# SamsungLabs/Metis

Hardware: NVIDIA H100
Metric: candidate plans evaluated/sec (higher is better)
Workload: dtype f64

## Files before the change

metis_b200/csrc/metis_eval.cuh:

```cuda
#pragma once

#include <stdint.h>
#include <string.h>
#include <math.h>

#include "../../include/metis_b200.h"

#if defined(__CUDACC__)
#define MB_HD __host__ __device__ __forceinline__
#define MB_HD_NOINLINE __host__ __device__ __noinline__
#else
#define MB_HD inline
#define MB_HD_NOINLINE inline
#endif

namespace metis {

constexpr int kH = 7;
constexpr double kMemCoef = 5.0;
constexpr uint8_t kDropped = 0xFF;

struct Tables {
    MetisProblem p;
    const int16_t *key_index;
    const double *lc;
    const double *mem;
    const double *exec_full;
    const double *fb_sync;
    const double *norm_lc;
    const double *type_memory, *bw_first, *bw_min;
    const uint8_t *run_type;
    const int32_t *run_end;
    const int32_t *q10_end;
    const double *dlay;
    const double *inv_exec;
    const double *ratio;
    const double *dpk;
    const double *pp_hidden;
    const double *pp_vocab;
    const double *psub;
    const double *dsub;
    const double *rsum;
};

constexpr int kDpk = 16;

struct DerivedLayout {
    int dlay, inv_exec, ratio, dpk, pp_hidden, pp_vocab, psub, dsub, total;
};

MB_HD DerivedLayout derived_layout(const MetisProblem &p) {
    DerivedLayout d;
    int o = 0;
    d.dlay = o; o += p.norm_len;
    d.inv_exec = o; o += p.num_keys;
    d.ratio = o; o += p.num_layers + 1;
    d.dpk = o; o += kDpk;
    d.pp_hidden = o; o += p.num_bs + 1;
    d.pp_vocab = o; o += (p.num_bs + 1) * p.num_tp;
    d.psub = o; o += (p.norm_len >= p.num_layers) ? kH * p.num_layers + 1 : 0;
    d.dsub = o; o += (p.norm_len >= p.num_layers) ? kH * p.num_layers : 0;
    d.total = o;
    return d;
}

MB_HD double derive_entry(const MetisProblem &p, const DerivedLayout &d, const double *norm_lc,
                          const double *exec_full, const double *bw_first, int i) {
    if (i < d.inv_exec) return norm_lc[i - d.dlay] / 7.0;
    if (i < d.ratio) return 1. / exec_full[i - d.inv_exec];
    if (i < d.dpk) return (double)(i - d.ratio) / (double)p.num_layers;
    const double bw = bw_first[0] * 1048576.0;
    if (i < d.pp_hidden) {
        const int dp = 1 << (i - d.dpk);
        return (double)(2 * (dp - 1)) / ((double)dp * bw);
    }
    if (i < d.pp_vocab) return (double)((int64_t)(i - d.pp_hidden) * p.sequence_length * p.hidden_size) / bw;
    if (i >= d.dsub) return norm_lc[(i - d.dsub) / kH] / 7.0;
    if (i >= d.psub) {
        const int j = i - d.psub, r = j / kH;
        double acc = 0.0;
        for (int t = 0; t < r; ++t) acc += norm_lc[t];
        return r < p.norm_len ? acc + norm_lc[r] * ((double)(j - r * kH) / 7.0) : acc;
    }
    const int e = i - d.pp_vocab;
    const int mbs = e / p.num_tp, tpc = e - mbs * p.num_tp;
    return ((double)((int64_t)mbs * p.sequence_length * p.vocab_size) / (double)(1 << tpc)) / bw;
}

MB_HD void bind_derived(Tables &T, const double *base) {
    const DerivedLayout d = derived_layout(T.p);
    T.dlay = base + d.dlay;
    T.inv_exec = base + d.inv_exec;
    T.ratio = base + d.ratio;
    T.dpk = base + d.dpk;
    T.pp_hidden = base + d.pp_hidden;
    T.pp_vocab = base + d.pp_vocab;
    T.psub = base + d.psub;
    T.dsub = base + d.dsub;
}

struct PlanDesc {
    uint32_t ordinal;
    int ns;
    int S;
    int label;
    int batches;
    const uint8_t *row;
    uint64_t geo;
};

MB_HD uint64_t pack_geo(int64_t row_offset, int S, int label, int ns, int div) {
    return (uint64_t)(row_offset & 0xFFFFFFFFLL) | ((uint64_t)((S - 1) & 0xFF) << 32) | ((uint64_t)((label - 1) & 0xFF) << 40) |
           ((uint64_t)(ns & 0xFF) << 48) | ((uint64_t)(div & 0xFF) << 56);
}

enum BalancerPath {
    kPathVerifyFailed = 0,
    kPathSeqForward = 1,
    kPathIrregular = 2,
    kPathMiddle = 3,
    kPathFirstGe = 4,
    kPathTail = 5,
    kPathVoteEnds = 6,
};

struct Serial {
    static constexpr bool kUniform = false;
    MB_HD void mark(int) const {}
    MB_HD void note(int) const {}
    MB_HD void converge() const {}
    MB_HD void rejoin(bool) {}
};
#if defined(__CUDACC__) && defined(METIS_PROFILE_PHASES)
constexpr int kBulkBatches = 31;
__device__ long long g_bulk_acc[32];
__shared__ long long s_bulk_t[32];
__shared__ int s_bulk_cur[32];
__device__ __forceinline__ void bulk_mark(unsigned group, int id) {
    __syncwarp(group);
    if ((int)(threadIdx.x & 31) == __ffs((int)group) - 1) {
        const int wi = threadIdx.x >> 5;
        const long long now = clock64();
        if (id == 1) atomicAdd((unsigned long long *)&g_bulk_acc[kBulkBatches], 1ULL);
        else atomicAdd((unsigned long long *)&g_bulk_acc[s_bulk_cur[wi] & 31], (unsigned long long)(now - s_bulk_t[wi]));
        s_bulk_cur[wi] = id;
        s_bulk_t[wi] = now;
    }
    __syncwarp(group);
}
#endif
#if defined(__CUDACC__)
struct Lockstep : Serial {
    unsigned mask;
    __device__ Lockstep() : mask(0xFFFFFFFFu) {}
    __device__ void converge() const { __syncwarp(mask); }
    __device__ void rejoin(bool p) { mask = __ballot_sync(0xFFFFFFFFu, p); }
#if defined(METIS_PROFILE_PHASES)
    __device__ void mark(int id) const { bulk_mark(__activemask(), id); }
#endif
};
#endif
struct SerialUniform : Serial {
    static constexpr bool kUniform = true;
};

constexpr uint64_t kOnes = 0x0101010101010101ULL;

constexpr uint16_t kBroke = 0x8000;
constexpr uint16_t kTaken = 0x4000;
constexpr uint16_t kPos = 0x3FFF;

template <int MAXS, int MAXL>
struct Scratch {
    double perf[MAXS];
    double capa[MAXS];
    double mstate[MAXS];
    double extra[MAXS];
    uint16_t fe[MAXS];
    uint16_t first[MAXS], lastl[MAXS], cnt[MAXS];
    uint16_t part[MAXS + 1];
    uint16_t rs[MAXS + 1];
    uint8_t gcode[MAXS];
    uint8_t tpc[MAXS];
    uint8_t lstk[MAXS];
    uint8_t got[MAXS];
    uint64_t ownerw[MAXL / 8 + 1];
    uint64_t subw[MAXL];
    static_assert(MAXL >= MAXS, "after the vote, subw holds one double per stage (CoopEvaluator's adjust and cost)");
};

MB_HD double py_sum_range(const double *x, int a, int b) {
    if (a >= b) return 0.0;
    double f = 0.0 + x[a];
    double c = 0.0;
    for (int i = a + 1; i < b; ++i) {
        const double v = x[i];
        const double t = f + v;
        if (fabs(f) >= fabs(v)) c += (f - t) + v;
        else c += (v - t) + f;
        f = t;
    }
    if (c != 0.0 && isfinite(c)) f += c;
    return f;
}

MB_HD_NOINLINE double py_sum_range_compact(const double *x, int a, int b) {
    if (a >= b) return 0.0;
    double f = 0.0 + x[a];
    double c = 0.0;
#pragma unroll 1
    for (int i = a + 1; i < b; ++i) {
        const double v = x[i];
        const double t = f + v;
        if (fabs(f) >= fabs(v)) c += (f - t) + v;
        else c += (v - t) + f;
        f = t;
    }
    if (c != 0.0 && isfinite(c)) f += c;
    return f;
}

template <class X>
MB_HD double sum_range(const double *x, int a, int b) {
    if constexpr (X::kUniform) return py_sum_range_compact(x, a, b);
    else return py_sum_range(x, a, b);
}

MB_HD void fill_range_sums(const double *row, int L, int a, double *out) {
    const int n = L + 1;
    double f = 0.0 + row[a];
    double c = 0.0;
    out[(size_t)(a + 1) * n + a] = f;
#if defined(__CUDA_ARCH__)
#pragma unroll 1
#endif
    for (int i = a + 1; i < L; ++i) {
        const double v = row[i];
        const double t = f + v;
        if (fabs(f) >= fabs(v)) c += (f - t) + v;
        else c += (v - t) + f;
        f = t;
        out[(size_t)(i + 1) * n + a] = (c != 0.0 && isfinite(c)) ? f + c : f;
    }
}
MB_HD int range_sum_tables(const MetisProblem &p) { return 2 * p.num_keys + 1; }
MB_HD const double *range_sum_row(const MetisProblem &p, int t, const double *mem, const double *lc, const double *norm) {
    if (t < p.num_keys) return mem + (size_t)t * p.lpad;
    if (t < 2 * p.num_keys) return lc + (size_t)(t - p.num_keys) * p.lpad;
    return p.norm_len >= p.num_layers ? norm : nullptr;
}

enum RangeTable { kRangeMem = 0, kRangeLc = 1, kRangeNorm = 2 };
template <class X>
MB_HD double range_sum(const Tables &T, int family, int key, const double *row, int a, int b) {
    if (a >= b) return 0.0;
    if (T.rsum && b <= T.p.num_layers) {
        const int n = T.p.num_layers + 1;
        const int t = family == kRangeMem ? key : family == kRangeLc ? T.p.num_keys + key : 2 * T.p.num_keys;
#if defined(__CUDA_ARCH__)
        return __ldg(&T.rsum[((size_t)t * n + b) * n + a]);
#else
        return T.rsum[((size_t)t * n + b) * n + a];
#endif
    }
    return sum_range<X>(row, a, b);
}

struct PySum {
    double f, c;
    int n;
    MB_HD PySum() : f(0.0), c(0.0), n(0) {}
    MB_HD void add(double v) {
        if (n == 0) { f = 0.0 + v; }
        else {
            const double t = f + v;
            if (fabs(f) >= fabs(v)) c += (f - t) + v;
            else c += (v - t) + f;
            f = t;
        }
        ++n;
    }
    MB_HD double result() const {
        double r = f;
        if (c != 0.0 && isfinite(c)) r += c;
        return r;
    }
};

MB_HD double pow2_neg(int k) {
    const uint64_t bits = (uint64_t)(1023 - k) << 52;
    double d;
    memcpy(&d, &bits, sizeof(d));
    return d;
}

MB_HD int type_of_rank(const Tables &T, int ns, int rank) {
    const int nt = T.p.num_types;
    const int32_t *end = T.run_end + ns * nt;
    const uint8_t *typ = T.run_type + ns * nt;
#pragma unroll 1
    for (int k = 0; k < nt; ++k)
        if (rank < end[k]) return typ[k];
    return typ[nt - 1];
}

MB_HD int type_of_q10(const Tables &T, int ns, int idx) {
    const int nt = T.p.num_types;
    const int32_t *end = T.q10_end + ns * nt;
    const uint8_t *typ = T.run_type + ns * nt;
#pragma unroll 1
    for (int k = 0; k < nt; ++k)
        if (idx < end[k]) return typ[k];
    return typ[nt - 1];
}

MB_HD int key_of(const Tables &T, int type, int tpc, int bs) {
    if (tpc >= T.p.num_tp || bs < 1 || bs > T.p.num_bs) return -1;
    return T.key_index[(type * T.p.num_tp + tpc) * T.p.num_bs + (bs - 1)];
}

template <int MAXS, int MAXL>
MB_HD int fwd_start(const Scratch<MAXS, MAXL> &w, int s) {
    if (s == 0) return 0;
    const uint16_t e = w.fe[s - 1];
    return (e & kPos) + ((e & kBroke) ? 1 : 0);
}

template <int MAXS, int MAXL>
MB_HD bool fwd_nonempty(const Scratch<MAXS, MAXL> &w, int s) {
    return (int)(w.fe[s] & kPos) > fwd_start(w, s);
}

MB_HD int popc64(uint64_t v) {
#if defined(__CUDA_ARCH__)
    return __popcll(v);
#else
    return __builtin_popcountll(v);
#endif
}
MB_HD int ctz64(uint64_t v) {
#if defined(__CUDA_ARCH__)
    return __ffsll((long long)v) - 1;
#else
    return __builtin_ctzll(v);
#endif
}
MB_HD int popc32(uint32_t v) {
#if defined(__CUDA_ARCH__)
    return __popc(v);
#else
    return __builtin_popcount(v);
#endif
}
MB_HD int ctz32(uint32_t v) {
#if defined(__CUDA_ARCH__)
    return __ffs((int)v) - 1;
#else
    return __builtin_ctz(v);
#endif
}
MB_HD int clz32(uint32_t v) {
#if defined(__CUDA_ARCH__)
    return __clz((int)v);
#else
    return __builtin_clz(v);
#endif
}
MB_HD int clz64(uint64_t v) {
#if defined(__CUDA_ARCH__)
    return __clzll((long long)v);
#else
    return __builtin_clzll(v);
#endif
}

MB_HD uint64_t swar_eq(uint64_t x, int c) {
    const uint64_t y = x ^ ((uint64_t)c * kOnes);
    const uint64_t lo7 = 0x7F7F7F7F7F7F7F7FULL;
    return ~((((y & lo7) + lo7) | y) | lo7);
}

MB_HD int swar_count(uint64_t x, int c) { return popc64(swar_eq(x, c) & 0x0080808080808080ULL); }

MB_HD int layer_owner(uint64_t v, bool plurality) {
    if (plurality) {
        int best = 0, own = (int)kDropped;
#pragma unroll 1
        for (int q = 0; q < kH; ++q) {
            const int cq = (int)((v >> (8 * q)) & 0xFF);
            const int n = swar_count(v, cq);
            if (n > best || (n == best && cq < own)) { best = n; own = cq; }
        }
        return own;
    }
    const int c3 = (int)((v >> 24) & 0xFF);
    if (swar_count(v, c3) * 2 > kH) return c3;
    const int c0 = (int)(v & 0xFF), c1 = (int)((v >> 8) & 0xFF), c2 = (int)((v >> 16) & 0xFF);
    if (swar_count(v, c0) * 2 > kH) return c0;
    if (c1 != c0 && swar_count(v, c1) * 2 > kH) return c1;
    if (c2 != c1 && c2 != c0 && swar_count(v, c2) * 2 > kH) return c2;
    return (int)kDropped;
}

template <int MAXS, int MAXL, class X>
MB_HD int balance_run(const Tables &T, int S, Scratch<MAXS, MAXL> &w, const X &x) {
    const int L = T.p.num_layers;
    if (T.p.norm_len < L) return METIS_FATAL_INDEX;
    const double *dlay = T.dlay;
    const double *lc = T.norm_lc;
    const int N = kH * L;
    const int lim = (N - 1 - kH) > 0 ? (N - 1 - kH) : 0;
    const int last = S - 1;
    int broken = METIS_FATAL_NONE;

#pragma unroll (X::kUniform ? 1 : 0)
    for (int s = 0; s < S; ++s) { w.got[s] = 0; w.cnt[s] = 0; }

    x.mark(10);
    int k = 0, sTop = -1;
    bool topSkip = false;
    if (S > 1) {
        int s = 0, j = 0;
        double c = w.perf[0];
#pragma unroll (X::kUniform ? 1 : 0)
        for (int r = 0; r + 1 < L; ++r) {
            const double d = dlay[r];
            const int nsub = (r == L - 2) ? kH - 1 : kH;
#pragma unroll
            for (int q = 0; q < kH; ++q) {
                if (q < nsub) {
                    if (s < last) {
                        if (c > d) {
                            c -= d;
                        } else {
                            w.capa[s] = c;
                            w.fe[s] = (uint16_t)(j | kBroke);
                            ++s;
                            c = w.perf[s];
                        }
                    }
                    ++j;
                }
            }
        }
        if (s < last) {
            x.note(kPathTail);
            w.capa[s] = c;
            w.fe[s] = (uint16_t)lim;
#pragma unroll (X::kUniform ? 1 : 0)
            for (int t = s + 1; t < last; ++t) { w.capa[t] = w.perf[t]; w.fe[t] = (uint16_t)lim; }
            k = lim;
            sTop = s;
        } else {
            k = (w.fe[last - 1] & kPos) + 1;
            sTop = last - 1;
            topSkip = true;
        }
    }

    x.mark(11);
    x.converge();
    int m;
    {
        double c = w.perf[last];
        const double dl = dlay[L - 1];
#pragma unroll (X::kUniform ? 1 : 0)
        for (int i = 0; i < kH; ++i) c -= dl;
        m = N - kH;
        int sp = S - 2;
#pragma unroll (X::kUniform ? 1 : 0)
        while (m > 0) {
            const int j = m - 1;
            bool un = (j >= k);
            if (!un) {
#pragma unroll (X::kUniform ? 1 : 0)
                while (sp >= 0 && (!(w.fe[sp] & kBroke) || (int)(w.fe[sp] & kPos) > j)) --sp;
                un = (sp >= 0 && (int)(w.fe[sp] & kPos) == j);
            }
            if (!un) break;
            const double d = dlay[j / kH];
            if (!(c > d)) break;
            c -= d;
            m = j;
            if (j < k) w.fe[sp] |= kTaken;
        }
        w.capa[last] = c;
    }

    x.mark(12);
    x.converge();
    {
        int start = 0;
#pragma unroll (X::kUniform ? 1 : 0)
        for (int s = 0; s < last; ++s) {
            const uint16_t e = w.fe[s];
            const int pos = e & kPos;
            const int next_start = pos + ((e & kBroke) ? 1 : 0);
            if ((e & (kBroke | kTaken)) != kBroke) { start = next_start; continue; }
            const int j = pos;
            int lo = 0;
            if (pos > start) {
                lo = s;
            } else {
                x.note(kPathIrregular);
#pragma unroll (X::kUniform ? 1 : 0)
                for (int u = s;; --u) {
                    if (u < s) {
                        const int t = w.lstk[u];
                        const bool above = (t == last) || (fwd_nonempty(w, t) && fwd_start(w, t) > j);
                        if (!above) { lo = t; break; }
                    }
                    if (fwd_nonempty(w, u)) { lo = u; break; }
                    if (u == 0) break;
                }
            }
            int hi = s + 1;
            if (hi < last && !((int)(w.fe[hi] & kPos) > next_start && !w.got[hi])) {
                ++hi;
#pragma unroll (X::kUniform ? 1 : 0)
                while (hi < last && (!fwd_nonempty(w, hi) || w.got[hi])) ++hi;
            }
            if (lo > hi) { broken = METIS_FATAL_SCRATCH; hi = lo; }
            int pick = lo;
            double best = w.capa[lo];
#pragma unroll (X::kUniform ? 1 : 0)
            for (int t = lo + 1; t <= hi; ++t)
                if (w.capa[t] > best) { best = w.capa[t]; pick = t; }
            w.capa[pick] -= dlay[j / kH];
            w.lstk[s] = (uint8_t)pick;
            w.got[pick] = 1;
            start = next_start;
        }
    }
    x.converge();
    const int nblk = m - k;
    if (nblk > 0) x.note(kPathMiddle);
    uint8_t *mid = reinterpret_cast<uint8_t *>(w.subw);
    {
        int below = -1;
#pragma unroll (X::kUniform ? 1 : 0)
        for (int t = 0; t < nblk; ++t) {
            const int j = k + t;
            int lo = 0;
            if (below >= 0) lo = below;
            else if (sTop >= 0) {
#pragma unroll (X::kUniform ? 1 : 0)
                for (int u = sTop;; --u) {
                    if (u < sTop || topSkip) {
                        const uint16_t eu = w.fe[u];
                        if ((eu & (kBroke | kTaken)) == kBroke) {
                            const int t2 = w.lstk[u];
                            if (t2 != last) { lo = t2; break; }
                        }
                    }
                    if (fwd_nonempty(w, u)) { lo = u; break; }
                    if (u == 0) break;
                }
            }
            int pick = lo;
            double best = w.capa[lo];
#pragma unroll (X::kUniform ? 1 : 0)
            for (int t2 = lo + 1; t2 <= last; ++t2)
                if (w.capa[t2] > best) { best = w.capa[t2]; pick = t2; }
            w.capa[pick] -= dlay[j / kH];
            if (pick != last) below = pick;
            mid[t] = (uint8_t)pick;
        }
    }

    x.mark(13);
    x.converge();
    if (k > 0) x.note(kPathVoteEnds);
    int t = 0, nxt = 0;
    uint16_t e = 0;
    if (k > 0) { e = w.fe[0]; nxt = (int)(e & kPos) + ((e & kBroke) ? 1 : 0); }
    const bool plurality = (T.p.corrected & METIS_FIX_Q5) != 0;
    int run_own = (int)kDropped, run_first = 0, run_len = 0;
#pragma unroll (X::kUniform ? 1 : 0)
    for (int r = 0; r < L; ++r) {
        int own = last;
        if (kH * r < m) {
            uint64_t v = 0xFF00000000000000ULL;
#pragma unroll
            for (int q = 0; q < kH; ++q) {
                const int j = kH * r + q;
                int st = last;
                if (j < k) {
#pragma unroll 1
                    while (nxt <= j) { ++t; e = w.fe[t]; nxt = (int)(e & kPos) + ((e & kBroke) ? 1 : 0); }
                    st = t;
                    if (nxt - 1 == j && (e & kBroke)) st = (e & kTaken) ? last : (int)w.lstk[t];
                } else if (j < m) {
                    st = mid[j - k];
                }
                v |= (uint64_t)(uint32_t)st << (8 * q);
            }
            own = layer_owner(v, plurality);
        }
        reinterpret_cast<uint8_t *>(w.ownerw)[r] = (uint8_t)own;
        {
            if (own == run_own) ++run_len;
            else {
                if (run_own != (int)kDropped) {
                    if (w.cnt[run_own] == 0) w.first[run_own] = (uint16_t)run_first;
                    w.lastl[run_own] = (uint16_t)(r - 1);
                    w.cnt[run_own] = (uint16_t)(w.cnt[run_own] + run_len);
                }
                run_own = own; run_first = r; run_len = 1;
            }
        }
    }
    if (run_own != (int)kDropped) {
        if (w.cnt[run_own] == 0) w.first[run_own] = (uint16_t)run_first;
        w.lastl[run_own] = (uint16_t)(L - 1);
        w.cnt[run_own] = (uint16_t)(w.cnt[run_own] + run_len);
    }
    x.mark(14);
    x.converge();
    uint8_t *owner = reinterpret_cast<uint8_t *>(w.ownerw);
    int top = 0x7FFFFFFF;
    double maxc = -INFINITY;
#pragma unroll (X::kUniform ? 1 : 0)
    for (int s = 0; s < S; ++s) {
        const double c = w.cnt[s] ? w.perf[s] - range_sum<X>(T, kRangeNorm, 0, lc, w.first[s], (int)w.lastl[s] + 1) : w.perf[s];
        w.capa[s] = c;
        if (c > maxc) { maxc = c; top = s; }
    }

    x.mark(15);
    x.converge();
#pragma unroll (X::kUniform ? 1 : 0)
    for (int n = 1; n <= 3; ++n) {
        if (top == 0x7FFFFFFF) top = 0;
        int nb = -1;
        double val = INFINITY;
        if (top - 1 >= 0 && w.capa[top - 1] < val) { nb = top - 1; val = w.capa[top - 1]; }
        if (top + 1 < S && w.capa[top + 1] < val) { nb = top + 1; }
        if (nb < 0 || w.cnt[nb] <= 1) break;
        const int layer = (top > nb) ? w.lastl[nb] : w.first[nb];
        const double dl = lc[layer];
        const double ntop = w.capa[top] - dl;
        const double nnb = w.capa[nb] + dl;
        double newmax = -INFINITY;
        int newtop = 0x7FFFFFFF;
#pragma unroll (X::kUniform ? 1 : 0)
        for (int t = 0; t < S; ++t) {
            const double v = (t == top) ? ntop : (t == nb) ? nnb : w.capa[t];
            if (v > newmax) { newmax = v; newtop = t; }
        }
        if (newmax > maxc) break;
        owner[layer] = (uint8_t)top;
        w.capa[top] = ntop;
        w.capa[nb] = nnb;
        if (top > nb) { int r = layer - 1; while (owner[r] != nb) --r; w.lastl[nb] = (uint16_t)r; }
        else          { int r = layer + 1; while (owner[r] != nb) ++r; w.first[nb] = (uint16_t)r; }
        if (w.cnt[top] == 0) { w.first[top] = (uint16_t)layer; w.lastl[top] = (uint16_t)layer; }
        else {
            if (layer < (int)w.first[top]) w.first[top] = (uint16_t)layer;
            if (layer > (int)w.lastl[top]) w.lastl[top] = (uint16_t)layer;
        }
        ++w.cnt[top];
        --w.cnt[nb];
        maxc = newmax;
        top = newtop;
    }

    x.mark(16);
    x.converge();
    w.part[0] = 0;
#pragma unroll (X::kUniform ? 1 : 0)
    for (int s = 0; s < S; ++s) w.part[s + 1] = (uint16_t)(w.part[s] + w.cnt[s]);
    return broken;
}

struct HSplit {
    int nruns;
    int type[METIS_MAX_TYPES];
    int n[METIS_MAX_TYPES];
    int base[METIS_MAX_TYPES];
    int plus[METIS_MAX_TYPES];
};

MB_HD_NOINLINE int partition_data(const Tables &T, int ns, int rank_lo, int count, int dp, int tpc, int bs,
                                  HSplit &out, uint32_t &aux, bool q10 = false) {
    const int gsz = count / dp;
    double perf[METIS_MAX_TYPES];
    PySum total;
    out.nruns = 0;
#pragma unroll 1
    for (int i = 0; i < dp; ++i) {
        const int t = q10 ? type_of_q10(T, ns, rank_lo + i * gsz) : type_of_rank(T, ns, rank_lo + i * gsz);
        if (out.nruns == 0 || out.type[out.nruns - 1] != t) {
            const int key = key_of(T, t, tpc, 1);
            if (key < 0) { aux = ((uint32_t)tpc << 16) | 1u; return METIS_FATAL_KEY_EXEC; }
            const double e = T.exec_full[key];
            if (e == 0.0) return METIS_FATAL_ZERODIV;
            out.type[out.nruns] = t;
            out.n[out.nruns] = 0;
            perf[out.nruns] = 1. / e;
            ++out.nruns;
        }
        ++out.n[out.nruns - 1];
        total.add(perf[out.nruns - 1]);
    }
    const double tot = total.result();
    double frac[METIS_MAX_TYPES];
    int assigned = 0;
#pragma unroll 1
    for (int r = 0; r < out.nruns; ++r) {
        const double v = (double)bs * (perf[r] / tot);
        const int b = (int)v;
        out.base[r] = b;
        out.plus[r] = 0;
        frac[r] = v - (double)b;
        assigned += b * out.n[r];
    }
    int rem = bs - assigned;
    bool used[METIS_MAX_TYPES];
#pragma unroll 1
    for (int r = 0; r < out.nruns; ++r) used[r] = false;
#pragma unroll 1
    for (int it = 0; it < out.nruns && rem > 0; ++it) {
        int pick = -1;
#pragma unroll 1
        for (int r = 0; r < out.nruns; ++r)
            if (!used[r] && (pick < 0 || frac[r] > frac[pick])) pick = r;
        used[pick] = true;
        const int g = rem < out.n[pick] ? rem : out.n[pick];
        out.plus[pick] = g;
        rem -= g;
    }
    if (rem > 0) return METIS_FATAL_SCRATCH;
    return METIS_FATAL_NONE;
}


struct TraceTap {
    double *demand;
    double *state;
    double cost[5];
};

MB_HD int halvings_of(const MetisProblem &p, int S, const uint8_t *gcode, const uint8_t *tpc, int bs_total) {
    int ltp = 0, lbs = 0;
    while ((2 << ltp) <= p.max_tp) ++ltp;
    while ((2 << lbs) <= p.max_bs) ++lbs;
    int u = 0;
#if defined(__CUDA_ARCH__)
#pragma unroll 1
#endif
    for (int s = 0; s < S; ++s) {
        const int g = gcode[s], t = tpc[s];
        int lm = 0;
        while ((2 << lm) <= (bs_total >> (g - t))) ++lm;
        int room = g - t;
        if (ltp - t < room) room = ltp - t;
        if (lbs - lm < room) room = lbs - lm;
        if (room > 0) u += room;
    }
    return u;
}

MB_HD double encode_error(int rc, uint32_t aux) { return rc ? (double)rc + (double)aux * 256.0 : 0.0; }
MB_HD int decode_error(double word, uint32_t &aux) {
    const uint64_t code = (uint64_t)word;
    aux = (uint32_t)(code >> 8);
    return (int)(code & 0xFF);
}

template <int MAXS, int MAXL, class X = Serial, bool ONE = false>
struct PlanEvaluator {
    const Tables &T;
    Scratch<MAXS, MAXL> &w;
    X x;
    PlanDesc pd;
    int bs_total;
    int nbad;
    uint32_t aux;
    TraceTap *tap;

    MB_HD PlanEvaluator(const Tables &t, Scratch<MAXS, MAXL> &s, const X &lanes = X())
        : T(t), w(s), x(lanes), bs_total(0), nbad(0), aux(0), tap(nullptr) {}

    MB_HD int group(int s) const { return 1 << w.gcode[s]; }
    MB_HD int dp_of(int s) const { return (1 << w.gcode[s]) >> w.tpc[s]; }

    MB_HD bool stage_bad(int g, int t) const {
        const int mbs = bs_total >> (g - t);
        return mbs == 0 || mbs > T.p.max_bs || (1 << t) > T.p.max_tp;
    }

    MB_HD int begin(const PlanDesc &plan) {
        pd = plan;
        if (pd.S > MAXS || T.p.num_layers > MAXL) return -1;
        bs_total = T.p.gbs / pd.batches;
        int lb = 0;
#pragma unroll (X::kUniform ? 1 : 0)
        while ((2 << lb) <= bs_total) ++lb;
        nbad = 0;
        int a = 0;
        for (int s = 0; s < pd.S; ++s) {
            const int g = pd.row[s];
            const int t = g > lb ? g - lb : 0;
            if (stage_bad(g, t)) { nbad = 1; return 0; }
            w.gcode[s] = (uint8_t)g;
            w.rs[s] = (uint16_t)a;
            a += 1 << g;
            w.tpc[s] = (uint8_t)t;
        }
        w.rs[pd.S] = (uint16_t)a;
        return nbad == 0 ? 1 : 0;
    }

    MB_HD bool next_strategy(bool have_state) {
        int pick = -1;
        if (have_state) {
            double best = 0.0;
#pragma unroll (X::kUniform ? 1 : 0)
            for (int s = 0; s < pd.S; ++s)
                if (w.gcode[s] != w.tpc[s] && (pick < 0 || w.mstate[s] < best)) { pick = s; best = w.mstate[s]; }
        } else {
            int best = -1;
#pragma unroll (X::kUniform ? 1 : 0)
            for (int s = 0; s < pd.S; ++s) {
                const int ldp = (int)w.gcode[s] - (int)w.tpc[s];
                if (ldp != 0 && ldp > best) { pick = s; best = ldp; }
            }
        }
        if (pick < 0) return false;
        const int g = w.gcode[pick], t = w.tpc[pick];
        nbad += (stage_bad(g, t + 1) ? 1 : 0) - (stage_bad(g, t) ? 1 : 0);
        w.tpc[pick] = (uint8_t)(t + 1);
        return true;
    }

    MB_HD bool valid() const { return nbad == 0; }

    MB_HD int halvings() const { return halvings_of(T.p, pd.S, w.gcode, w.tpc, bs_total); }

    MB_HD double memory_capacity(int a, int b) const {
        const int nt = T.p.num_types;
        if (ONE || nt == 1) return T.type_memory[0] * (double)(b - a);
        const int32_t *end = T.run_end + pd.ns * nt;
        const uint8_t *typ = T.run_type + pd.ns * nt;
        PySum acc;
        int lo = 0;
#pragma unroll (X::kUniform ? 1 : 0)
        for (int k = 0; k < nt; ++k) {
            const int hi = end[k];
            const int x = (a > lo ? a : lo), y = (b < hi ? b : hi);
            if (y > x) acc.add(T.type_memory[typ[k]] * (double)(y - x));
            lo = hi;
        }
        return acc.result();
    }

    MB_HD int replica_perf_cost(int type, int tpc, int h, double &out) {
        double acc = 0.;
#pragma unroll (X::kUniform ? 1 : 0)
        for (int bit = 30; bit >= 0; --bit) {
            const int piece = 1 << bit;
            if (!(h & piece)) continue;
            const int key = key_of(T, type, tpc, piece);
            if (key < 0) { aux = ((uint32_t)tpc << 16) | (uint32_t)piece; return METIS_FATAL_KEY_EXEC; }
            acc += T.exec_full[key];
        }
        out = acc;
        return 0;
    }

    MB_HD_NOINLINE int hetero_performance(int a, int b, int dp, int tpc, double &p) {
        HSplit hs;
        int rc = partition_data(T, pd.ns, a, b - a, dp, tpc, bs_total, hs, aux);
        if (rc) return rc;
        double mx = -INFINITY;
#pragma unroll (X::kUniform ? 1 : 0)
        for (int r = 0; r < hs.nruns; ++r) {
            double c;
            if (hs.plus[r] > 0) {
                rc = replica_perf_cost(hs.type[r], tpc, hs.base[r] + 1, c);
                if (rc) return rc;
                if (c > mx) mx = c;
            }
            if (hs.plus[r] < hs.n[r]) {
                rc = replica_perf_cost(hs.type[r], tpc, hs.base[r], c);
                if (rc) return rc;
                if (c > mx) mx = c;
            }
        }
        p = (mx != 0.0) ? 1. / mx : 0.0;
        return 0;
    }

    MB_HD int rank_start(int s) const { return w.rs[s]; }


    MB_HD int stage_performance(int s, double &p) {
        const int g = w.gcode[s], tpc = w.tpc[s];
        const int a = rank_start(s), b = a + (1 << g);
        int ta = 0, tb = 0;
        if (!(ONE || T.p.num_types == 1)) { ta = type_of_rank(T, pd.ns, a); tb = type_of_rank(T, pd.ns, b - 1); }
        p = 0.0;
        if (ta != tb) return hetero_performance(a, b, 1 << (g - tpc), tpc, p);
        const int bs = bs_total >> (g - tpc);
        const int key = key_of(T, ta, tpc, bs);
        if (key < 0) { aux = ((uint32_t)tpc << 16) | (uint32_t)bs; return METIS_FATAL_KEY_EXEC; }
        if (T.exec_full[key] == 0.0) return METIS_FATAL_ZERODIV;
        p = T.inv_exec[key];
        return 0;
    }

    MB_HD int stage_memory(int s, double &demand, double &state) {
        const bool one_type = ONE || T.p.num_types == 1;
        const bool own_type = (T.p.corrected & METIS_FIX_Q6) != 0;
        const int g = w.gcode[s], tpc = w.tpc[s];
        const int a = rank_start(s), b = a + (1 << g);
        int rc = 0;
        demand = 0.001;
        if (!ONE && own_type) {
            rc = memory_demand_own_type(s, demand);
        } else if (T.p.q10_devices < T.p.total_devices && !own_type && b > T.p.q10_devices) {
            aux = 0;
            rc = METIS_FATAL_INDEX;
        } else if (one_type || type_of_q10(T, pd.ns, a) == type_of_q10(T, pd.ns, b - 1)) {
            const int bs = bs_total >> (g - tpc);
            const int key = key_of(T, T.run_type[pd.ns * T.p.num_types], tpc, bs);
            if (key < 0) { aux = ((uint32_t)tpc << 16) | (uint32_t)bs; rc = METIS_FATAL_KEY_MEMORY; }
            else demand += range_sum<X>(T, kRangeMem, key, T.mem + (size_t)key * T.p.lpad, w.part[s], w.part[s + 1]) * kMemCoef;
        } else {
            rc = hetero_memory_demand(s, T.run_type[pd.ns * T.p.num_types], demand);
        }
        state = memory_capacity(a, b) - demand;
        return rc;
    }

    MB_HD void stage_adjust(int s, double &avail, double &adj, double &extra) const {
        const double c = w.perf[s], md = w.extra[s];
        const double mc = memory_capacity(rank_start(s), rank_start(s) + group(s));
        if (mc > md) {
            adj = c;
            avail = (c * mc / md) - c;
            extra = 0.0;
        } else {
            avail = 0.0;
            adj = c * (mc / md) * 0.9;
            extra = c - adj;
        }
    }

    MB_HD bool stage_time(int s, double &len) {
        const bool one_type = ONE || T.p.num_types == 1;
        const int g = w.gcode[s], tpc = w.tpc[s];
        const int a = one_type ? 0 : rank_start(s), b = a + (1 << g);
        const int la = w.part[s], lb = w.part[s + 1];
        const int ldp = g - tpc;
        const int ta = one_type ? 0 : type_of_rank(T, pd.ns, a);
        const int tb = one_type ? 0 : type_of_rank(T, pd.ns, b - 1);
        len = 0.0;
        if (ta != tb) return hetero_exec_cost(a, b, 1 << ldp, tpc, la, lb, len) != 0;
        const int key = key_of(T, ta, tpc, bs_total >> ldp);
        if (key < 0) return true;
        len = range_sum<X>(T, kRangeLc, key, T.lc + (size_t)key * T.p.lpad, la, lb);
        return false;
    }

    MB_HD void stage_terms(int s, int nstage, double &pp, double &dpc, double &upd) const {
        const int per = T.p.devices_per_node;
        const int Lm = T.p.num_layers;
        const bool ubw = T.p.uniform_bw != 0;
        const int g = w.gcode[s], tpc = w.tpc[s];
        const int la = w.part[s], lb = w.part[s + 1];
        const int ldp = g - tpc;
        const int mbs = bs_total >> ldp;
        const double inv_tp = pow2_neg(tpc);
        pp = 0.0;
        if (s < nstage - 1) {
            if (ubw) {
                pp = (lb == Lm - 1) ? T.pp_vocab[mbs * T.p.num_tp + tpc] : T.pp_hidden[mbs];
            } else {
                double act;
                if (lb == Lm - 1)
                    act = (double)((int64_t)mbs * T.p.sequence_length * T.p.vocab_size) * inv_tp;
                else
                    act = (double)((int64_t)mbs * T.p.sequence_length * T.p.hidden_size);
                pp = act / (bw_of_node_range(rank_start(s) / per, (rank_start(s + 2) - 1) / per) * 1048576.0);
            }
        }
        int ntr = lb - la;
        double params = 0.0;
        if (la == 0) { params += T.p.input_params * inv_tp; --ntr; }
        if (lb == Lm) { params += T.p.output_params * inv_tp; --ntr; }
        params += T.p.transformer_params * inv_tp * (double)ntr;
        if (ubw) dpc = T.dpk[ldp] * params;
        else {
            const int dp = 1 << ldp;
            dpc = (double)(2 * (dp - 1)) / ((double)dp * (dp_bandwidth(rank_start(s), dp, 1 << tpc) * 1048576.0)) * params;
        }
        upd = T.p.optimizer_time * inv_tp * T.ratio[lb - la];
    }


    MB_HD int compute_performance() {
        PySum total;
        int rc = 0;
#pragma unroll (X::kUniform ? 1 : 0)
        for (int s = 0; s < pd.S; ++s) {
            double p;
            rc = stage_performance(s, p);
            if (rc) break;
            w.perf[s] = p;
            total.add(p);
        }
        x.converge();
        if (rc) return rc;
        const double tot = total.result();
        if (tot == 0.0) return METIS_FATAL_ZERODIV;
#pragma unroll (X::kUniform ? 1 : 0)
        for (int s = 0; s < pd.S; ++s) w.perf[s] = w.perf[s] / tot;
        return 0;
    }

    MB_HD_NOINLINE int hetero_memory_demand(int s, int type0, double &demand) {
        const int la = w.part[s], lb = w.part[s + 1], tpc = w.tpc[s];
        HSplit hs;
        const int rc = partition_data(T, pd.ns, 0, T.p.q10_devices, dp_of(s), tpc, bs_total, hs, aux, true);
        if (rc) return rc;
#pragma unroll (X::kUniform ? 1 : 0)
        for (int r = 0; r < hs.nruns; ++r)
#pragma unroll (X::kUniform ? 1 : 0)
            for (int i = 0; i < hs.n[r]; ++i) {
                const int h = hs.base[r] + (i < hs.plus[r] ? 1 : 0);
#pragma unroll (X::kUniform ? 1 : 0)
                for (int bit = 30; bit >= 0; --bit) {
                    const int piece = 1 << bit;
                    if (!(h & piece)) continue;
                    const int key = key_of(T, type0, tpc, piece);
                    if (key < 0) { aux = ((uint32_t)tpc << 16) | (uint32_t)piece; return METIS_FATAL_KEY_MEMORY; }
                    demand += range_sum<X>(T, kRangeMem, key, T.mem + (size_t)key * T.p.lpad, la, lb) * kMemCoef;
                }
            }
        return 0;
    }

    MB_HD_NOINLINE int memory_demand_own_type(int s, double &demand) {
        const int la = w.part[s], lb = w.part[s + 1], tpc = w.tpc[s], g = w.gcode[s];
        const int a = rank_start(s), b = a + (1 << g);
        const int ta = type_of_rank(T, pd.ns, a), tb = type_of_rank(T, pd.ns, b - 1);
        if (ta == tb) {
            const int bs = bs_total >> (g - tpc);
            const int key = key_of(T, ta, tpc, bs);
            if (key < 0) { aux = ((uint32_t)tpc << 16) | (uint32_t)bs; return METIS_FATAL_KEY_MEMORY; }
            demand += range_sum<SerialUniform>(T, kRangeMem, key, T.mem + (size_t)key * T.p.lpad, la, lb) * kMemCoef;
            return 0;
        }
        HSplit hs;
        const int rc = partition_data(T, pd.ns, a, b - a, 1 << (g - tpc), tpc, bs_total, hs, aux);
        if (rc) return rc;
        double worst = 0.0;
#pragma unroll 1
        for (int r = 0; r < hs.nruns; ++r)
#pragma unroll 1
            for (int v = 0; v < 2; ++v) {
                const int cntv = v ? hs.plus[r] : hs.n[r] - hs.plus[r];
                const int h = hs.base[r] + v;
                if (cntv <= 0 || h == 0) continue;
                double need = 0.0;
#pragma unroll 1
                for (int bit = 30; bit >= 0; --bit) {
                    const int piece = 1 << bit;
                    if (!(h & piece)) continue;
                    const int key = key_of(T, hs.type[r], tpc, piece);
                    if (key < 0) { aux = ((uint32_t)tpc << 16) | (uint32_t)piece; return METIS_FATAL_KEY_MEMORY; }
                    need += range_sum<SerialUniform>(T, kRangeMem, key, T.mem + (size_t)key * T.p.lpad, la, lb) * kMemCoef;
                }
                if (need > worst) worst = need;
            }
        demand += worst;
        return 0;
    }

    MB_HD_NOINLINE int adjust_performance() {
        const int S = pd.S;
        double need = 0.;
        PySum avail_sum;
#pragma unroll (X::kUniform ? 1 : 0)
        for (int s = 0; s < S; ++s) {
            double av, adj, extra;
            stage_adjust(s, av, adj, extra);
            w.capa[s] = av;
            w.mstate[s] = adj;
            w.extra[s] = 0.;
            need += extra;
            avail_sum.add(av);
        }
        if (avail_sum.result() < need) return 1;
        int guard = 0;
#pragma unroll (X::kUniform ? 1 : 0)
        while (need > 0.01) {
            PySum tot;
#pragma unroll (X::kUniform ? 1 : 0)
            for (int s = 0; s < S; ++s) tot.add(w.capa[s] > 0.001 ? w.perf[s] : 0.0);
            const double tmp_total = tot.result();
#pragma unroll (X::kUniform ? 1 : 0)
            for (int s = 0; s < S; ++s) {
                const double av = w.capa[s];
                const double ratio = av > 0.001 ? w.perf[s] / tmp_total : 0.0;
                const double want = need * ratio;
                const double give = want > av ? av : want;
                w.extra[s] += give;
                w.capa[s] -= give;
                need -= give;
            }
            if (++guard > 4096) return -METIS_FATAL_HANG;
        }
#pragma unroll (X::kUniform ? 1 : 0)
        for (int s = 0; s < S; ++s) w.perf[s] = w.extra[s] + w.mstate[s];
        return 0;
    }

    MB_HD int memory_phase(int attempt) {
        const int S = pd.S;
        bool oom = false;
        int rc = 0;
#pragma unroll (X::kUniform ? 1 : 0)
        for (int s = 0; s < S; ++s) {
            double md, state;
            rc = stage_memory(s, md, state);
            if (rc) break;
            w.extra[s] = md;
            w.mstate[s] = state;
            if (state < 0) oom = true;
            if (tap) { tap->demand[s] = md; tap->state[s] = state; }
        }
        x.converge();
        if (rc) return -rc;
        if (!oom) return 1;
        if (attempt >= 3) return 0;
        x.mark(21);
        const int adj = adjust_performance();
        if (adj < 0) return adj;
        return adj == 1 ? 0 : 2;
    }

    template <class Sink>
    MB_HD_NOINLINE int partition_layer(Sink &sink) {
#pragma unroll (X::kUniform ? 1 : 0)
        for (int attempt = 1; attempt <= 3; ++attempt) {
            sink.balancer_run();
            const int rc = balance_run<MAXS, MAXL>(T, pd.S, w, x);
            if (rc) return -rc;
            const int r = memory_phase(attempt);
            if (r == 1) return attempt;
            if (r <= 0) return r;
        }
        return 0;
    }

    MB_HD double bw_of_node_range(int n0, int n1) const {
        const int per = T.p.devices_per_node;
        if (n0 == n1) return T.bw_first[type_of_q10(T, pd.ns, n0 * per)];
        double slow = INFINITY;
        const int nt = T.p.num_types;
        const int32_t *end = T.q10_end + pd.ns * nt;
        const uint8_t *typ = T.run_type + pd.ns * nt;
        int lo = 0;
#pragma unroll (X::kUniform ? 1 : 0)
        for (int k = 0; k < nt; ++k) {
            const int hi = end[k];
            if (hi > lo && n0 * per < hi && (n1 + 1) * per > lo) {
                const double v = T.bw_min[typ[k]];
                if (v < slow) slow = v;
            }
            lo = hi;
        }
        return slow;
    }

    MB_HD double dp_bandwidth(int a, int dp, int tp) const {
        const int per = T.p.devices_per_node;
        double slow = INFINITY;
#pragma unroll (X::kUniform ? 1 : 0)
        for (int d = 0; d < dp; ++d) {
            const int n0 = (a + d) / per;
            int nlast = n0;
            bool multi = false;
            double gmin = INFINITY;
            int tprev = -1;
#pragma unroll (X::kUniform ? 1 : 0)
            for (int i = 0; i < tp; ++i) {
                const int node = (a + d + i * dp) / per;
                if (node != nlast) { multi = true; nlast = node; }
                const int t = type_of_q10(T, pd.ns, node * per);
                if (t != tprev) { const double v = T.bw_min[t]; if (v < gmin) gmin = v; tprev = t; }
            }
            const double bw = multi ? gmin : T.bw_first[type_of_q10(T, pd.ns, n0 * per)];
            if (bw < slow) slow = bw;
        }
        return slow;
    }

    MB_HD_NOINLINE int hetero_exec_cost(int a, int b, int dp, int tpc, int la, int lb, double &len) {
        HSplit hs;
        uint32_t dummy;
        if (partition_data(T, pd.ns, a, b - a, dp, tpc, bs_total, hs, dummy)) return 1;
        len = -INFINITY;
#pragma unroll (X::kUniform ? 1 : 0)
        for (int r = 0; r < hs.nruns; ++r)
#pragma unroll (X::kUniform ? 1 : 0)
            for (int v = 0; v < 2; ++v) {
                const int cntv = v ? hs.plus[r] : hs.n[r] - hs.plus[r];
                const int h = hs.base[r] + v;
                if (cntv <= 0 || h == 0) continue;
                double acc = 0.;
#pragma unroll (X::kUniform ? 1 : 0)
                for (int bit = 30; bit >= 0; --bit) {
                    const int piece = 1 << bit;
                    if (!(h & piece)) continue;
                    if (piece > T.p.max_bs) return 1;
                    const int key = key_of(T, hs.type[r], tpc, piece);
                    if (key < 0) return 1;
                    acc += range_sum<X>(T, kRangeLc, key, T.lc + (size_t)key * T.p.lpad, la, lb);
                }
                if (acc > len) len = acc;
            }
        return 0;
    }

    MB_HD int fb_sync_cost(int a, int b, int tpc, int mbs, double &out) const {
        const int nt = T.p.num_types;
        const int32_t *end = T.run_end + pd.ns * nt;
        const uint8_t *typ = T.run_type + pd.ns * nt;
        double mx = -INFINITY;
        int lo = 0;
#pragma unroll (X::kUniform ? 1 : 0)
        for (int k = 0; k < nt; ++k) {
            const int hi = end[k];
            if ((a > lo ? a : lo) < (b < hi ? b : hi)) {
                const int key = key_of(T, typ[k], tpc, mbs);
                if (key < 0) return 1;
                const double v = T.fb_sync[key];
                if (v == 0.0) return 1;
                if (v > mx) mx = v;
            }
            lo = hi;
        }
        out = mx;
        return 0;
    }

    MB_HD int get_cost(double &cost_out) {
        const bool one_type = ONE || T.p.num_types == 1;
        const int nstage = pd.label < pd.S ? pd.label : pd.S;
        if (T.p.q10_devices < T.p.total_devices && rank_start(nstage) > T.p.q10_devices) return 1;
        bool bad = false;
        PySum lens_sum;
        double max_len = -INFINITY;
#pragma unroll (X::kUniform ? 1 : 0)
        for (int s = 0; s < nstage; ++s) {
            double len;
            if (stage_time(s, len)) bad = true;
            lens_sum.add(len);
            if (len > max_len) max_len = len;
        }
        if (bad) return 1;
        double max_upd = -INFINITY, max_dp = -INFINITY;
        double pp_cost = 0., fb_sync = 0.;
#pragma unroll (X::kUniform ? 1 : 0)
        for (int s = 0; s < nstage; ++s) {
            double pp, dpc, upd;
            stage_terms(s, nstage, pp, dpc, upd);
            if (s < nstage - 1) pp_cost += pp;
            if (dpc > max_dp) max_dp = dpc;
            if (upd > max_upd) max_upd = upd;
        }
        {
            const int s = nstage - 1;
            const int a = one_type ? 0 : rank_start(s), b = a + group(s);
            double v;
            if (fb_sync_cost(a, b, w.tpc[s], bs_total >> (w.gcode[s] - w.tpc[s]), v)) return 1;
            fb_sync = v * (double)pd.batches;
        }
        const double exec = ((double)(pd.batches - 1) * max_len) + lens_sum.result();
        const double bg = T.p.batch_generator * (double)pd.batches;
        cost_out = exec + fb_sync + max_upd + max_dp + pp_cost + bg;
        if (tap) { tap->cost[0] = exec; tap->cost[1] = fb_sync; tap->cost[2] = max_upd; tap->cost[3] = max_dp; tap->cost[4] = pp_cost; }
        return 0;
    }

    template <class Sink>
    MB_HD_NOINLINE void run(const PlanDesc &plan, Sink &sink, int only_step = -1) {
        const int ok = begin(plan);
        if (ok < 0) { sink.fatal(plan.ordinal, METIS_FATAL_SCRATCH, 0); return; }
        if (ok == 0) return;
        bool started = false, have_state = false;
        int nrep = 0, step = 0;
#pragma unroll (X::kUniform ? 1 : 0)
        for (;;) {
            if (nrep == 1) return;
            int attempt = 0;
#pragma unroll (X::kUniform ? 1 : 0)
            for (;;) {
                if (!started) started = true;
                else if (!next_strategy(have_state)) return;
                if (!valid()) continue;
                sink.partition_call();
                int rc = compute_performance();
                if (rc) { sink.fatal(pd.ordinal, rc, aux); return; }
                attempt = partition_layer(sink);
                if (attempt < 0) { sink.fatal(pd.ordinal, -attempt, aux); return; }
                have_state = attempt > 0;
                if (attempt > 0) break;
            }
            nrep = attempt;
            double cost;
            if (get_cost(cost) == 0) sink.emit(pd, step, nrep, cost, w.tpc, w.part);
            else sink.keyerror();
            if (only_step >= 0 && step == only_step) return;
            ++step;
        }
    }
};

template <int MAXS, int MAXL, bool ONE, class X = Serial, class Sink>
MB_HD bool first_task(const Tables &T, Scratch<MAXS, MAXL> &w, Sink &sink, bool has, const PlanDesc &plan, int &chain_hint,
                      int &resume) {
    PlanEvaluator<MAXS, MAXL, X, ONE> ev(T, w);
    bool cont = false;
    sink.phase(1);
    if (has) {
        const int ok = ev.begin(plan);
        if (ok < 0) sink.fatal(plan.ordinal, METIS_FATAL_SCRATCH, 0);
        has = ok == 1;
    }
    ev.x.rejoin(has);
    if (has) {
        sink.partition_call();
        const int rc = ev.compute_performance();
        if (rc) { sink.fatal(plan.ordinal, rc, ev.aux); has = false; }
    }
    sink.phase(2);
    ev.x.rejoin(has);
    if (has) {
        sink.balancer_run();
        const int rc = balance_run<MAXS, MAXL>(T, plan.S, w, ev.x);
        if (rc) { sink.fatal(plan.ordinal, rc, ev.aux); has = false; }
    }
    sink.phase(3);
    ev.x.rejoin(has);
    bool costing = false;
    if (has) {
        const int r = ev.memory_phase(1);
        if (r < 0) sink.fatal(plan.ordinal, -r, ev.aux);
        else if (r != 1) {
            cont = true;
            chain_hint = ev.halvings();
            resume = r == 2 ? 2 : 3;
        } else costing = true;
    }
    sink.phase(4);
    ev.x.rejoin(costing);
    if (costing) {
        double cost;
        if (ev.get_cost(cost) == 0) sink.emit(plan, 0, 1, cost, w.tpc, w.part);
        else sink.keyerror();
    }
    sink.phase(0);
    ev.x.rejoin(true);
    return cont;
}

MB_HD int homo_cost(const Tables &T, int type, int dp, int pp, int tp, int mbs, int gbs, double &cost_out,
                    int &oom, TraceTap *tap = nullptr) {
    const int L = T.p.num_layers;
    const int per = T.p.devices_per_node;
    int tpc = 0;
#pragma unroll 1
    while ((1 << tpc) < tp) ++tpc;
    const int key = ((1 << tpc) == tp) ? key_of(T, type, tpc, mbs) : -1;
    if (key < 0) return 1;
    const int num_mbs = gbs / mbs / dp;
    (void)type;
    const double intra = T.p.node0_bandwidth;
    const double inter = T.p.node0_bandwidth;
    const int base = (L - 2) / pp, rem = (L - 2) % pp;
    PySum lens_sum;
    double max_len = -INFINITY, max_params = -INFINITY, max_mem = -INFINITY;
    double pp_cost = 0., fb_sync = 0.;
    int a = 0;
#pragma unroll 1
    for (int s = 0; s < pp; ++s) {
        int count = base + ((s >= 1 && s <= rem) ? 1 : 0) + (s == 0 ? 1 : 0) + (s == pp - 1 ? 1 : 0);
        const int b = a + count;
        const double len = py_sum_range(T.lc + (size_t)key * T.p.lpad, a, b);
        lens_sum.add(len);
        if (len > max_len) max_len = len;
        PySum ps;
#pragma unroll 1
        for (int r = a; r < b && r < L; ++r) {
            const double v = (r == 0) ? T.p.input_params / (double)tp
                           : (r == L - 1) ? T.p.output_params / (double)tp
                           : T.p.transformer_params / (double)tp;
            ps.add(v);
        }
        const double sp = ps.result();
        if (sp > max_params) max_params = sp;
        const double sm = py_sum_range(T.mem + (size_t)key * T.p.lpad, a, b);
        if (sm > max_mem) max_mem = sm;
        if (tap) tap->demand[s] = sm;
        if (s == pp - 1) {
            const double v = T.fb_sync[key];
            if (v == 0.0) return 1;
            fb_sync = v * (double)num_mbs;
        } else {
            double act;
            if (b == L - 1) act = (double)((int64_t)mbs * T.p.sequence_length * T.p.vocab_size) / (double)tp;
            else act = (double)((int64_t)mbs * T.p.sequence_length * T.p.hidden_size);
            double bw = intra;
#pragma unroll 1
            for (int d = 0; d < dp; ++d)
#pragma unroll 1
                for (int t = 0; t < tp; ++t) {
                    const int r0 = s * dp * tp + d * tp + t, r1 = r0 + dp * tp;
                    if (r0 / per != r1 / per) bw = inter;
                }
            pp_cost += act / (bw * 1048576.0);
        }
        a = b;
    }
    oom = (T.p.node0_memory < max_mem) ? 1 : 0;
    const double exec = ((double)(num_mbs - 1) * max_len) + lens_sum.result();
    const double upd = T.p.optimizer_time / (double)pp / (double)tp;
    double bw = intra;
#pragma unroll 1
    for (int p = 0; p < pp; ++p)
        if ((p * dp * tp) / per != ((p + 1) * dp * tp - 1) / per) bw = inter;
    const double dpc = (double)(2 * (dp - 1)) / ((double)dp * (bw * 1048576.0)) * max_params;
    const double bg = T.p.batch_generator * (double)num_mbs;
    cost_out = exec + fb_sync + upd + dpc + pp_cost + bg;
    if (tap) { tap->cost[0] = exec; tap->cost[1] = fb_sync; tap->cost[2] = upd; tap->cost[3] = dpc; tap->cost[4] = pp_cost; }
    return 0;
}

}
```

Baseline: 210.5 million.

## Prefetch stage capacities and vote slots ahead in balance loops

Adds a small lookahead buffer (Ahead) so that the next perf values and fe/lstk vote slots are loaded into registers before they are needed. The stage-assignment loop becomes branch-free selects, with a noinline fallback used when more than two stages advance within one layer. The run-length accounting uses a register bitmask of seen stages instead of reading w.cnt. The aim is to take dependent local-memory loads off the critical path and cut divergence, at the cost of extra registers and some redundant loads.

Result: no change. 211.5 million (median of 6 runs) (+0.5%).

```diff
diff --git a/metis_b200/csrc/metis_eval.cuh b/metis_b200/csrc/metis_eval.cuh
--- a/metis_b200/csrc/metis_eval.cuh
+++ b/metis_b200/csrc/metis_eval.cuh
@@ -402,6 +402,26 @@
     return (int)kDropped;
 }
 
+template <class V>
+struct Ahead {
+    V n1, n2, f3, f4;
+    template <class At> MB_HD void init(const At &at) { n1 = at(1); n2 = at(2); f3 = at(3); f4 = at(4); }
+    template <class At> MB_HD void advance(int moved, int i, const At &at) {
+        if (moved == 1) { n1 = n2; n2 = f3; }
+        else if (moved == 2) { n1 = f3; n2 = f4; }
+        else if (moved > 2) { n1 = at(i + 1); n2 = at(i + 2); }
+        if (moved > 0) { f3 = at(i + 3); f4 = at(i + 4); }
+    }
+    MB_HD V next(int moved) const { return moved == 0 ? n1 : n2; }
+};
+
+template <class At>
+MB_HD_NOINLINE auto ahead_miss(const At &at, int i) -> decltype(at(i)) { return at(i); }
+
+struct VoteSlot {
+    uint32_t fe, lk;
+};
+
 template <int MAXS, int MAXL, class X>
 MB_HD int balance_run(const Tables &T, int S, Scratch<MAXS, MAXL> &w, const X &x) {
     const int L = T.p.num_layers;
@@ -420,28 +440,35 @@
     int k = 0, sTop = -1;
     bool topSkip = false;
     if (S > 1) {
-        int s = 0, j = 0;
+        int s = 0, sh = 0, j = 0;
         double c = w.perf[0];
+        const auto perf_at = [&](int i) { return w.perf[i < last ? i : last]; };
+        Ahead<double> pa;
+        pa.init(perf_at);
+        double d = dlay[0];
 #pragma unroll (X::kUniform ? 1 : 0)
         for (int r = 0; r + 1 < L; ++r) {
-            const double d = dlay[r];
+            const double dn = dlay[r + 1];
             const int nsub = (r == L - 2) ? kH - 1 : kH;
+            pa.advance(s - sh, s, perf_at);
+            sh = s;
 #pragma unroll
             for (int q = 0; q < kH; ++q) {
                 if (q < nsub) {
-                    if (s < last) {
-                        if (c > d) {
-                            c -= d;
-                        } else {
-                            w.capa[s] = c;
-                            w.fe[s] = (uint16_t)(j | kBroke);
-                            ++s;
-                            c = w.perf[s];
-                        }
+                    const bool open = s < last;
+                    const bool close = open && !(c > d);
+                    if (close) {
+                        w.capa[s] = c;
+                        w.fe[s] = (uint16_t)(j | kBroke);
                     }
+                    double pn = pa.next(s - sh);
+                    if (close && s - sh > 1) pn = ahead_miss(perf_at, s + 1);
+                    c = close ? pn : open ? c - d : c;
+                    s += close;
                     ++j;
                 }
             }
+            d = dn;
         }
         if (s < last) {
             x.note(kPathTail);
@@ -571,25 +598,52 @@
     x.mark(13);
     x.converge();
     if (k > 0) x.note(kPathVoteEnds);
-    int t = 0, nxt = 0;
-    uint16_t e = 0;
-    if (k > 0) { e = w.fe[0]; nxt = (int)(e & kPos) + ((e & kBroke) ? 1 : 0); }
+    const int tmax = last > 0 ? last - 1 : 0;
+    const auto slot_of = [&](int i) { return VoteSlot{w.fe[i], w.lstk[i]}; };
+    const auto slot_at = [&](int i) { return slot_of(i < tmax ? i : tmax); };
+    const auto slot_end = [](uint32_t e) { return (int)(e & kPos) + ((e & kBroke) ? 1 : 0); };
+    int t = 0, th = 0, nxt = 0;
+    VoteSlot e{0, 0};
+    Ahead<VoteSlot> sa;
+    if (k > 0) { e = slot_of(0); nxt = slot_end(e.fe); sa.init(slot_at); }
     const bool plurality = (T.p.corrected & METIS_FIX_Q5) != 0;
     int run_own = (int)kDropped, run_first = 0, run_len = 0;
+    uint64_t seen0 = 0, seen1 = 0;
+    const auto close_run = [&](int lastl) {
+        bool seen;
+        if constexpr (MAXS > 64) seen = run_own < 64 ? (seen0 >> run_own) & 1 : (seen1 >> (run_own - 64)) & 1;
+        else seen = (seen0 >> run_own) & 1;
+        if (seen) w.cnt[run_own] = (uint16_t)(w.cnt[run_own] + run_len);
+        else {
+            w.first[run_own] = (uint16_t)run_first;
+            w.cnt[run_own] = (uint16_t)run_len;
+            if (MAXS <= 64 || run_own < 64) seen0 |= 1ULL << (run_own & 63);
+            else seen1 |= 1ULL << (run_own & 63);
+        }
+        w.lastl[run_own] = (uint16_t)lastl;
+    };
 #pragma unroll (X::kUniform ? 1 : 0)
     for (int r = 0; r < L; ++r) {
         int own = last;
         if (kH * r < m) {
+            sa.advance(t - th, t, slot_at);
+            th = t;
             uint64_t v = 0xFF00000000000000ULL;
 #pragma unroll
             for (int q = 0; q < kH; ++q) {
                 const int j = kH * r + q;
                 int st = last;
                 if (j < k) {
-#pragma unroll 1
-                    while (nxt <= j) { ++t; e = w.fe[t]; nxt = (int)(e & kPos) + ((e & kBroke) ? 1 : 0); }
+                    const bool adv = nxt <= j;
+                    VoteSlot en = sa.next(t - th);
+                    if (adv && t - th > 1) en = ahead_miss(slot_at, t + 1);
+                    e = adv ? en : e;
+                    t += adv;
+                    nxt = slot_end(e.fe);
+#pragma unroll 1
+                    while (nxt <= j) { ++t; e = slot_of(t); nxt = slot_end(e.fe); }
                     st = t;
-                    if (nxt - 1 == j && (e & kBroke)) st = (e & kTaken) ? last : (int)w.lstk[t];
+                    if (nxt - 1 == j && (e.fe & kBroke)) st = (e.fe & kTaken) ? last : (int)e.lk;
                 } else if (j < m) {
                     st = mid[j - k];
                 }
@@ -598,23 +652,13 @@
             own = layer_owner(v, plurality);
         }
         reinterpret_cast<uint8_t *>(w.ownerw)[r] = (uint8_t)own;
-        {
-            if (own == run_own) ++run_len;
-            else {
-                if (run_own != (int)kDropped) {
-                    if (w.cnt[run_own] == 0) w.first[run_own] = (uint16_t)run_first;
-                    w.lastl[run_own] = (uint16_t)(r - 1);
-                    w.cnt[run_own] = (uint16_t)(w.cnt[run_own] + run_len);
-                }
-                run_own = own; run_first = r; run_len = 1;
-            }
-        }
-    }
-    if (run_own != (int)kDropped) {
-        if (w.cnt[run_own] == 0) w.first[run_own] = (uint16_t)run_first;
-        w.lastl[run_own] = (uint16_t)(L - 1);
-        w.cnt[run_own] = (uint16_t)(w.cnt[run_own] + run_len);
-    }
+        if (own == run_own) ++run_len;
+        else {
+            if (run_own != (int)kDropped) close_run(r - 1);
+            run_own = own; run_first = r; run_len = 1;
+        }
+    }
+    if (run_own != (int)kDropped) close_run(L - 1);
     x.mark(14);
     x.converge();
     uint8_t *owner = reinterpret_cast<uint8_t *>(w.ownerw);
```
